# parthjaggi/flow

Hardware: AMD Instinct MI355X
Metric: env-steps/sec (higher is better)
Workload: dtype mixed

## Files before the change

flow_amd/csrc/flowsim.hip:

```cpp
#include "flowsim_sim.h"
#include "flowsim_learn.h"
#include "flowsim_es.h"

#include <cmath>

namespace fsim {

int validate(const fs_config* c) {
  if (!c) return fail(FS_ERR_INVALID, "fs_create: cfg is NULL");
  if (c->struct_size != sizeof(fs_config))
    return fail(FS_ERR_INVALID, "fs_create: struct_size mismatch (header/library out of sync)");
  if (c->abi_version != FS_ABI_VERSION) return fail(FS_ERR_INVALID, "fs_create: abi_version mismatch");
  if (c->precision != FS_F32 && c->precision != FS_F64 && c->precision != FS_MIXED && c->precision != FS_F16S)
    return fail(FS_ERR_INVALID, "fs_create: bad precision");
  if (c->precision == FS_F16S && (c->network != FS_NET_MERGE || c->num_vehicles > 64))
    return fail(FS_ERR_UNSUPPORTED, "fs_create: FS_F16S (half state, float32 integrator) is built for FS_NET_MERGE "
                                    "(k_steps_open, <= 64 vehicle slots)");
  if (c->precision == FS_MIXED && (c->network == FS_NET_MERGE || c->network == FS_NET_BOTTLENECK)) {
  } else if (c->precision == FS_MIXED) {
    const bool fig8 = c->network == FS_NET_FIGURE_EIGHT;
    const char* why = nullptr;
    if ((c->network != FS_NET_RING && !fig8) || c->num_lanes > 1) why = "network (single-lane ring or figure eight)";
    else if (c->env == FS_ENV_MULTI_WAVE_ATTENUATION_PO)
      why = "env (FS_ENV_MULTI_WAVE_ATTENUATION_PO is built for FS_F32, and for FS_F64 on the generic kernel)";
// ... 211 lines not shown
      const double x = c->init_pos[size_t(r) * c->num_vehicles + i];
      if (!(x >= 0) || !(x < L)) return fail(FS_ERR_INVALID, "fs_create: init_pos outside [0, length)");
    }
  }
  return FS_OK;
}

template <typename T>
int create_typed(const fs_config* cfg, fs_handle* out) {
  Sim<T>* s = new (std::nothrow) Sim<T>();
  if (!s) return fail(FS_ERR_HIP, "fs_create: out of host memory");
  s->cfg = *cfg;
  s->mixed = cfg->precision == FS_MIXED;
  s->f16s = cfg->precision == FS_F16S;
  s->veh.assign(cfg->vehicles, cfg->vehicles + cfg->num_vehicles);
  if (cfg->num_segments > 0) s->segs.assign(cfg->segments, cfg->segments + cfg->num_segments);
  if (cfg->obs_perm) s->obs_perm.assign(cfg->obs_perm, cfg->obs_perm + cfg->num_vehicles);
  if (cfg->network == FS_NET_MERGE || cfg->network == FS_NET_BOTTLENECK) {
    if (cfg->num_inflows > 0) s->inflows.assign(cfg->inflows, cfg->inflows + cfg->num_inflows);
    s->init_alive.assign(cfg->init_alive, cfg->init_alive + size_t(cfg->num_replicas) * cfg->num_vehicles);
    if (cfg->env == FS_ENV_BOTTLENECK_DV) {
      s->obs_cells.assign(cfg->obs_cells, cfg->obs_cells + cfg->num_obs_cells);
      if (cfg->num_rl > 0) s->act_cells.assign(cfg->act_cells, cfg->act_cells + cfg->num_rl);
    }
  }
  s->obs_dim = (cfg->env == FS_ENV_WAVE_ATTENUATION_PO) ? 3
               : (cfg->env == FS_ENV_WAVE_ATTENUATION_PO_MA) ? 3 * cfg->num_rl
               : (cfg->env == FS_ENV_MULTI_WAVE_ATTENUATION_PO) ? 3
               : (cfg->env == FS_ENV_ACCEL_PO_MA) ? 6 * cfg->num_rl
               : (cfg->env == FS_ENV_BOTTLENECK_DV) ? 4 * cfg->num_obs_cells + 1
               : (cfg->env == FS_ENV_BOTTLENECK) ? 1
               : (cfg->env == FS_ENV_MERGE_PO || cfg->env == FS_ENV_MERGE_MA)
                     ? 5 * cfg->num_rl
                     : (cfg->env == FS_ENV_LANE_CHANGE_ACCEL_PO)
                           ? (4 * (cfg->num_lanes < 1 ? 1 : cfg->num_lanes) + 1) * cfg->num_rl
                           : (cfg->env == FS_ENV_LANE_CHANGE_ACCEL ? 3 : 2) * cfg->num_vehicles;
  if (s->obs_dim < 1) s->obs_dim = 1;
  s->act_dim = cfg->num_rl * ((cfg->env == FS_ENV_LANE_CHANGE_ACCEL || cfg->env == FS_ENV_LANE_CHANGE_ACCEL_PO) ? 2 : 1);
  int seg = 8;
  while (seg < cfg->num_vehicles) seg <<= 1;
  s->seg = seg;
  hipError_t e = hipSetDevice(cfg->device);
  if (e == hipSuccess) e = hipStreamCreateWithFlags(&s->own_stream, hipStreamNonBlocking);
  if (e != hipSuccess) {
    delete s;
    return fail(FS_ERR_HIP, std::string("fs_create: no usable HIP device: ") + hipGetErrorString(e));
  }
  s->stream = s->own_stream;
  {
    const std::pair<const char*, bool SimBase::*> switches[] = {
        {"FLOWSIM_FORCE_GENERIC", &SimBase::force_generic}, {"FLOWSIM_NO_FASTDIV", &SimBase::no_fastdiv},
        {"FLOWSIM_NO_LOOP_KERNEL", &SimBase::no_loop_kernel}, {"FLOWSIM_NO_LOOP_FULL", &SimBase::no_loop_full},
        {"FLOWSIM_NO_RING_RL", &SimBase::no_ring_rl}, {"FLOWSIM_NO_QUEUE", &SimBase::no_queue},
        {"FLOWSIM_NO_PAIR", &SimBase::no_pair}, {"FLOWSIM_NO_MASK_SKIP", &SimBase::no_mask_skip},
        {"FLOWSIM_SNAPSHOT_COPIES", &SimBase::snap_copies}};
    for (const auto& sw : switches) {
      const char* v = std::getenv(sw.first);
      s->*sw.second = v && v[0] == '1';
    }
  }
  int rc = s->init();
  if (rc == FS_OK) {
    hipError_t e2 = hipStreamSynchronize(s->stream);
    if (e2 != hipSuccess) rc = fail(FS_ERR_HIP, std::string("fs_create: ") + hipGetErrorString(e2));
  }
  if (rc != FS_OK) {
    for (void* p : s->allocs) (void)hipFree(p);
    (void)hipStreamDestroy(s->own_stream);
    delete s;
    return rc;
  }
  s->cfg.vehicles = nullptr;
  s->cfg.ring_length = nullptr;
  s->cfg.init_pos = nullptr;
  s->cfg.init_vel = nullptr;
  s->cfg.init_lane = nullptr;
  s->cfg.segments = nullptr;
  s->cfg.inflows = nullptr;
  s->cfg.init_alive = nullptr;
  s->cfg.obs_cells = nullptr;
  s->cfg.obs_perm = nullptr;
  s->cfg.act_cells = nullptr;
  *out = reinterpret_cast<fs_handle>(static_cast<SimBase*>(s));
  return FS_OK;
}

inline SimBase* S(fs_handle h) { return reinterpret_cast<SimBase*>(h); }

struct DeviceGuard {
  int prev = -1;
  bool switched = false;
  explicit DeviceGuard(int want) {
    if (hipGetDevice(&prev) == hipSuccess && prev != want) switched = hipSetDevice(want) == hipSuccess;
  }
  ~DeviceGuard() {
    if (switched) (void)hipSetDevice(prev);
  }
};

}

using namespace fsim;

extern "C" {

int fs_abi_version(void) { return FS_ABI_VERSION; }

// ... 740 lines not shown
```

flow_amd/csrc/flowsim_launch.h:

```cpp
#pragma once
#include "flowsim_sim.h"
#ifdef FS_PART_QUEUE
#include "flowsim_queue.h"
#include "flowsim_dropq.h"
#endif

namespace fsim {

#ifdef FS_PART_QUEUE
  template <typename T>
  int Sim<T>::launch_queue(const StepArgs& a) {
    const bool po = dv.env == FS_ENV_MERGE_PO;
    const bool noise = (dv.flags & fs::FLAG_HAS_NOISE) != 0, act = a.actions != nullptr && (po || ov.ma_apply_actions != 0);
    const auto k = pick(noise, [&](auto NZ) {
      return pick(act, [&](auto ACT) {
        return pick(po, [&](auto PO) { return &fs::k_merge_queue<NZ, ACT, false, PO>; });
      });
    });
    last_kernel = "k_merge_queue";
    hipLaunchKernelGGL(k, dim3(dv.R), dim3(64), 0, stream, dv, ov, qc, a.num_steps, a.actions, a.act_stride, a.obs, a.rew,
                       a.done, a.obs_every_step, fs::PolicyView{}, static_cast<float*>(nullptr), static_cast<float*>(nullptr),
                       0);
    return launched();
  }
// ... 141 lines not shown
    } else if constexpr (std::is_same<T, float>::value) {
      const auto MC = std::false_type();
      k = !ma_head ? single(MC) : dv.env == FS_ENV_ACCEL_PO_MA ? kernel(Int<3>(), MC) : kernel(Int<2>(), MC);
    } else {
      k = single(std::false_type());
    }
    if constexpr (std::is_same<T, float>::value) {
      if (dv.env == FS_ENV_MULTI_WAVE_ATTENUATION_PO) k = kernel(Int<4>(), std::false_type());
    }
    last_kernel = dv.env == FS_ENV_MULTI_WAVE_ATTENUATION_PO ? "k_ring_pair<MultiRing>" : ma_head ? (dv.env == FS_ENV_ACCEL_PO_MA ? "k_ring_pair<AccelMA>" : "k_ring_pair<POMA>")
                          : (po ? "k_ring_pair<PO>" : "k_ring_pair<Accel>");
    const int waves = (dv.R + (64 / ROW) - 1) / (64 / ROW);
    hipLaunchKernelGGL(k, dim3((waves + 3) / 4), dim3(256), 0, stream, dv, a.num_steps, a.mask, a.actions, a.act_stride,
                       a.obs, a.rew, a.done, a.obs_every_step);
    return launched();
  }

  template <typename T>
  int Sim<T>::launch_obs_mixed(const StepArgs& a) {
    if constexpr (std::is_same<T, double>::value) {
      const int n = dv.R * dv.N;
      last_kernel = "k_obs_mixed";
      hipLaunchKernelGGL((fs::k_obs_mixed<T>), dim3((n + 255) / 256), dim3(256), 0, stream, dv, a.obs);
      return launched();
    } else {
      return fail(FS_ERR_UNSUPPORTED, "k_obs_mixed is a float64 kernel");
    }
  }

  template <typename T>
  template <int SEG>
  int Sim<T>::launch_pair(const StepArgs& a) {
    constexpr int ROW = SEG >= 16 ? SEG / 2 : 8;
    const bool fd = fastdiv_ok(), bc = neg_speed_possible, sm = speed_mode_any;
    const bool noise = std::is_same<T, float>::value && (dv.flags & fs::FLAG_HAS_NOISE);
    auto clamped = [&](auto SM, auto NZ) {
      return delta4 && fd && !bc ? &fs::k_rollout_pair<T, ROW, true, true, false, SM, NZ>
                                 : &fs::k_rollout_pair<T, ROW, false, false, true, SM, NZ>;
    };
    decltype(&fs::k_rollout_pair<T, ROW, false, false, true>) k = nullptr;
    if (noise) {
      if constexpr (std::is_same<T, float>::value) k = pick(sm, [&](auto SM) { return clamped(SM, std::true_type()); });
    } else if (sm) {
      k = clamped(std::true_type(), std::false_type());
    } else {
      k = pick(bc, [&](auto BC) {
        return delta4 && fd ? &fs::k_rollout_pair<T, ROW, true, true, BC>
                            : delta4 ? &fs::k_rollout_pair<T, ROW, true, false, BC> : &fs::k_rollout_pair<T, ROW, false, false, BC>;
      });
    }
    last_kernel = noise ? (sm ? "k_rollout_pair+speed_mode+noise" : "k_rollout_pair+noise")
                        : (sm ? "k_rollout_pair+speed_mode" : "k_rollout_pair");
    const int waves = (dv.R + (64 / ROW) - 1) / (64 / ROW);
    hipLaunchKernelGGL(k, dim3((waves + 3) / 4), dim3(256), 0, stream, dv, a.num_steps, a.obs, a.rew, a.done);
    return launched();
  }

  template <typename T>
  template <int SEG>
  int Sim<T>::launch_idm(const StepArgs& a) {
    constexpr int RPW = 64 / SEG;
    const bool fd = fastdiv_ok();
    const auto k = pick(neg_speed_possible, [&](auto BC) {
      return delta4 && fd ? &fs::k_rollout_idm<T, SEG, true, true, BC>
                          : delta4 ? &fs::k_rollout_idm<T, SEG, true, false, BC> : &fs::k_rollout_idm<T, SEG, false, false, BC>;
    });
    last_kernel = "k_rollout_idm";
    const int waves = (dv.R + RPW - 1) / RPW;
    hipLaunchKernelGGL(k, dim3((waves + 7) / 8), dim3(512), 0, stream, dv, a.num_steps, a.obs, a.rew, a.done, d_dump);
    return launched();
  }

  template <typename T>
  template <int SEG>
  int Sim<T>::launch_k_steps(const StepArgs& a) {
    constexpr int RPW = 64 / SEG;
    auto k = &fs::k_steps<T, SEG, 0, 0>;
    last_kernel = "k_steps";
    if (fast_ok(a)) {
      k = &fs::k_steps<T, SEG, 1, 0>;
      last_kernel = "k_steps<FAST>";
    } else if ((dv.flags & fs::FLAG_IDM_SET) && !force_generic) {
      k = &fs::k_steps<T, SEG, 0, 1>;
      last_kernel = "k_steps<CSET>";
    }
    hipLaunchKernelGGL(k, dim3((dv.R + RPW - 1) / RPW), dim3(64), 0, stream, dv, a.num_steps, a.mask, a.actions,
                       a.act_stride, a.obs, a.rew, a.done, a.obs_every_step);
    return launched();
  }

  template <typename T>
  int Sim<T>::launch_policy_act(const fs::PolicyView& pv, int n_ag, const float* obs_in, float* act, float* logp) {
    last_kernel = "k_policy_act";
    const bool merge = dv.env == FS_ENV_MERGE_MA;
    hipLaunchKernelGGL(fs::k_policy_act<16>, dim3((dv.R * 16 + 255) / 256), dim3(256), 0, stream, pv, dv.R, n_ag, dv.rep0,
                       obs_in, act, logp, merge ? static_cast<const int*>(dv.lane) : nullptr,
                       merge ? static_cast<const int*>(dv.ctrl) : nullptr,
                       merge ? static_cast<const int*>(dv.rl_index) : nullptr, dv.N);
    return launched();
  }

  template <typename T>
  int Sim<T>::launch_policy_row16(const fs::PolicyView& pv, int num_steps, int reset_done, float* obs, float* act,
                                  float* logp, float* rew, uint8_t* done) {
    const bool fast = ringrl_fast_ok();
    auto kernel = [&](auto H) {
// ... 89 lines not shown
```

flow_amd/csrc/flowsim_pair.h:

```cpp
#pragma once
#include "flowsim_kernels.h"

namespace fs {

typedef float f2 __attribute__((ext_vector_type(2)));
typedef unsigned u2v __attribute__((__vector_size__(8)));

enum : int { DPP_ROW_NEWBCAST0 = 0x150, DPP_ROW_NEWBCAST8 = 0x158 };

__device__ __forceinline__ f2 fma2(f2 a, f2 b, f2 c) { return __builtin_elementwise_fma(a, b, c); }
__device__ __forceinline__ f2 splat(float a) { return f2{a, a}; }

__device__ __forceinline__ f2 pk_mul(f2 a, f2 b) { return a * b; }
__device__ __forceinline__ f2 pk_add(f2 a, f2 b) { return a + b; }
__device__ __forceinline__ f2 pk_sub(f2 a, f2 b) { return a - b; }
__device__ __forceinline__ f2 pk_fma(f2 a, f2 b, f2 c) { return fma2(a, b, c); }
__device__ __forceinline__ f2 pk_fnma(f2 a, f2 b, f2 c) { return fma2(-a, b, c); }
__device__ __forceinline__ float nonneg_else(float x, float y) {
  const unsigned a = __builtin_bit_cast(unsigned, x), b = __builtin_bit_cast(unsigned, y);
  return __builtin_bit_cast(float, min(a, b));
}

template <int ROW>
__device__ __forceinline__ float next_a(float v, bool last, int lane) {
// ... 385 lines not shown
                                                    const MixedConsts& c) {
  unsigned long long sa, sb;
  asm volatile(
      "v_add_f64 v[134:135], v[114:115], -%[L]\n"
      "v_add_f64 v[136:137], v[116:117], -%[L]\n"
      "v_cmp_gt_i32_e64 %[sa], 0, v135\n"
      "v_cmp_gt_i32_e64 %[sb], 0, v137\n"
      "s_nop 0\n"
      "v_cndmask_b32_e64 v114, v134, v114, %[sa]\n"
      "v_cndmask_b32_e64 v115, v135, v115, %[sa]\n"
      "v_cndmask_b32_e64 v116, v136, v116, %[sb]\n"
      "v_cndmask_b32_e64 v117, v137, v117, %[sb]\n"
      "v_mul_f64 v[120:121], v[114:115], %[rcL]\n"
      "v_mul_f64 v[122:123], v[116:117], %[rcL]\n"
      "v_add_f64 v[134:135], v[116:117], -v[114:115]\n"
      "v_cvt_f32_f64_e32 v144, v[120:121]\n"
      "v_cvt_f32_f64_e32 v145, v[122:123]\n"
      "v_add_f64 v[126:127], v[134:135], %[L]\n"
      "v_mov_b32_dpp v130, v114 row_shl:1 row_mask:0xf bank_mask:0xf bound_ctrl:1\n"
      "v_mov_b32_dpp v131, v115 row_shl:1 row_mask:0xf bank_mask:0xf bound_ctrl:1\n"
      "v_mov_b32_dpp v132, v114 row_newbcast:0 row_mask:0xf bank_mask:0xf\n"
      "v_mov_b32_dpp v133, v115 row_newbcast:0 row_mask:0xf bank_mask:0xf\n"
      "v_cmp_gt_i32_e64 %[sa], 0, v135\n"
      "v_cndmask_b32_e64 v130, v130, v132, %[last]\n"
      "v_cndmask_b32_e64 v131, v131, v133, %[last]\n"
      "v_add_f64 v[136:137], v[130:131], -v[116:117]\n"
      "v_cndmask_b32_e64 v134, v134, v126, %[sa]\n"
      "v_cndmask_b32_e64 v135, v135, v127, %[sa]\n"
      "v_cndmask_b32_e64 v156, 0, %[Llo], %[sa]\n"
      "v_cndmask_b32_e64 v157, 0, %[Lhi], %[sa]\n"
      "v_add_f64 v[132:133], v[136:137], %[L]\n"
      "v_cmp_gt_i32_e64 %[sb], 0, v137\n"
      "v_add_f64 v[134:135], v[134:135], -%[lenb]\n"
      "v_cvt_f32_f64_e32 v140, v[134:135]\n"
      "v_cndmask_b32_e64 v136, v136, v132, %[sb]\n"
      "v_cndmask_b32_e64 v137, v137, v133, %[sb]\n"
      "v_cndmask_b32_e64 v158, 0, %[Llo], %[sb]\n"
      "v_cndmask_b32_e64 v159, 0, %[Lhi], %[sb]\n"
      "v_add_f64 v[136:137], v[136:137], -%[lennext]\n"
      "v_cvt_f32_f64_e32 v141, v[136:137]\n"
      "v_pk_add_f32 v[126:127], v[140:141], %[gap2] neg_lo:[0,1] neg_hi:[0,1]\n"
      "v_cmp_nlt_f32_e64 %[sa], |v140|, %[c1e3]\n"
      "v_cmp_nlt_f32_e64 %[sb], |v141|, %[c1e3]\n"
      "v_min_f32_e32 %[ct], v126, v127\n"
      "v_cndmask_b32_e64 v140, %[c1e3], v140, %[sa]\n"
      "v_cndmask_b32_e64 v141, %[c1e3], v141, %[sb]\n"
      : "+{v[114:115]}"(XA), "+{v[116:117]}"(XB), "+{v[140:141]}"(H), "+{v[144:145]}"(OX), "+{v[156:157]}"(WA),
        "+{v[158:159]}"(WB), [ct] "+v"(ct), [sa] "=&s"(sa), [sb] "=&s"(sb)
      : [L] "v"(c.L), [Llo] "v"(c.L_lo), [Lhi] "v"(c.L_hi), [rcL] "v"(c.rc_L), [gap2] "v"(c.gap2), [lenb] "v"(c.len_b),
        [lennext] "v"(c.len_next), [c1e3] "v"(c.c1e3), [last] "s"(c.last_mask)
      : "v120", "v121", "v122", "v123", "v126", "v127", "v130", "v131", "v132", "v133", "v134", "v135", "v136", "v137");
}

template <typename T, int ROW, bool DELTA4, bool FASTDIV, bool BADCHK, bool SM = false, bool NOISE = false>
__global__ __launch_bounds__(256) void k_rollout_pair(DevView<T> s, int num_steps, float* __restrict__ obs,
                                                      float* __restrict__ rew, uint8_t* __restrict__ done) {
  constexpr bool MIXED = sizeof(T) == 8;
  static_assert(!(NOISE && MIXED), "FS_MIXED has no noise form (its C twin cannot reproduce the hardware's log / cos)");
  constexpr bool ASM = ROW == 16 && DELTA4 && FASTDIV && !BADCHK;
  constexpr int RPW = 64 / ROW;
  constexpr int PERIOD = ROW < 16 ? ROW : 16;
  const int lane = threadIdx.x & 63;
  const int wave = (blockIdx.x * blockDim.x + threadIdx.x) >> 6;
  const int row = lane / ROW;
  const int k = lane % ROW;
  const int r = wave * RPW + row;
  const int N = s.N;
  const int LP = N >> 1;
  const bool rvalid = r < s.R;
  const bool valid = rvalid && k < LP;
  const int rr = rvalid ? r : s.R - 1;
  const int kk = k < LP ? k : LP - 1;
  const bool last = (kk == LP - 1);
  const int iA = 2 * kk, iB = iA + 1;
  const size_t idx = size_t(rr) * N + iA;

  f2 p[6];
#pragma unroll
  for (int q = 0; q < 6; ++q) p[q] = f2{float(s.p[q * N + iA]), float(s.p[q * N + iB])};
  const T lenB = s.length[iB];
  const T len_nextA = next_a<ROW>(T(s.length[iA]), last, lane);
  const T base_len = s.ring_len[rr];
  const T L = base_len + T(4) * s.jlen;
  int tcount = s.time[rr];
  uint32_t nctr = NOISE ? s.noise_ctr[rr] : 0u;
  const f2 sigma = NOISE ? f2{float(s.noise[iA]), float(s.noise[iB])} : f2{0.0f, 0.0f};
  const bool noisyA = NOISE && sigma.x > 0.0f, noisyB = NOISE && sigma.y > 0.0f;
  float gA[4] = {0.0f, 0.0f, 0.0f, 0.0f}, gB[4] = {0.0f, 0.0f, 0.0f, 0.0f};
  if constexpr (NOISE) {
    if ((nctr & 3u) != 0u) {
      gauss4<float>(s.seed_lo, s.seed_hi, s.rep0 + uint32_t(rr), uint32_t(iA), nctr >> 2, gA, s.noise_exact != 0);
      gauss4<float>(s.seed_lo, s.seed_hi, s.rep0 + uint32_t(rr), uint32_t(iB), nctr >> 2, gB, s.noise_exact != 0);
      for (uint32_t q = 0; q < (nctr & 3u); ++q) {
        gA[0] = gA[1]; gA[1] = gA[2]; gA[2] = gA[3];
        gB[0] = gB[1]; gB[1] = gB[2]; gB[2] = gB[3];
      }
    }
  }

  const float dt = float(s.dt), ramp = float(s.ramp);
  const f2 two_sqrt_ab = {2.0f * tsqrt(p[2].x * p[3].x), 2.0f * tsqrt(p[2].y * p[3].y)};
  const f2 rc_v0 = {1.0f / p[0].x, 1.0f / p[0].y}, rc_ab = {1.0f / two_sqrt_ab.x, 1.0f / two_sqrt_ab.y};
  const float Lf = float(L);
  const f2 L2 = splat(Lf), rc_L2 = splat(1.0f / Lf), one = splat(1.0f), dt2 = splat(dt), ramp2 = splat(ramp);
  const f2 gap2 = splat(float(s.crash_gap)), m100 = splat(-100.0f);
  const f2 vmask = splat(valid ? 1.0f : 0.0f), tvm = splat(valid ? -float(s.target_velocity) : 0.0f);
  const double ms64 = double(s.max_speed), rc_ms64 = 1.0 / ms64;
  const double L64 = double(L), rc_L64 = 1.0 / L64, dt64 = double(s.dt), ramp64 = double(s.ramp);

  f2 x, v;
  double xdA = 0, xdB = 0, vdA = 0, vdB = 0;
  if (MIXED) {
    xdA = double(s.pos[idx]); xdB = double(s.pos[idx + 1]);
    vdA = double(s.vel[idx]); vdB = double(s.vel[idx + 1]);
    v = f2{float(vdA), float(vdB)};
    x = f2{0.0f, 0.0f};
  } else {
    x = f2{float(s.pos[idx]), float(s.pos[idx + 1])};
    v = f2{float(s.vel[idx]), float(s.vel[idx + 1])};
  }
// ... 27 lines not shown
  mc.p0 = p[0]; mc.p1 = p[1]; mc.p2 = p[2]; mc.p5 = p[5]; mc.rc_v0 = rc_v0; mc.tsab = two_sqrt_ab; mc.rc_ab = rc_ab;
  mc.one = one; mc.gap2 = gap2; mc.vmask = vmask; mc.tvm = tvm; mc.c1e3 = 1e-3f; mc.dt = dt64; mc.ramp = ramp64;
  mc.L = L64; mc.rc_L = rc_L64; mc.rc_ms = rc_ms64; mc.len_b = double(lenB); mc.len_next = double(len_nextA);
  mc.zero = 0.0; mc.last_mask = pc.last_mask;
  {
    const unsigned long long Lb = __builtin_bit_cast(unsigned long long, L64);
    mc.L_lo = unsigned(Lb); mc.L_hi = unsigned(Lb >> 32);
    mc.thr = mc.L_hi < 0x457CED91u ? mc.L_hi : 0x457CED91u;
  }
  double wA = 0.0, wB = 0.0;
  if constexpr (ASM && MIXED) {
    asm volatile("" : "+v"(mc.dt), "+v"(mc.ramp), "+v"(mc.one), "+v"(mc.zero), "+v"(mc.rc_ms), "+v"(mc.c1e3), "+v"(mc.gap2));
    const double xn = next_a<ROW>(xdA, last, lane);
    wA = xdB - xdA < 0.0 ? L64 : 0.0;
    wB = xn - xdB < 0.0 ? L64 : 0.0;
    h.x = tabs(h.x) < 1e-3f ? 1e-3f : h.x;
    h.y = tabs(h.y) < 1e-3f ? 1e-3f : h.y;
  }
  SumoPair sc{};
  double floor0A = 0, floor0B = 0, adtA = 0, adtB = 0, ddtA = 0, ddtB = 0;
  if constexpr (SM) {
    const int mA = s.speed_mode[iA], mB = s.speed_mode[iB];
    const float maA = float(s.max_accel[iA]), maB = float(s.max_accel[iB]);
    const float mdA = float(s.max_decel[iA]), mdB = float(s.max_decel[iB]);
    sc.tau = f2{float(s.sumo_tau[iA]), float(s.sumo_tau[iB])};
    sc.min_gap = f2{float(s.sumo_min_gap[iA]), float(s.sumo_min_gap[iB])};
    sc.maxa = f2{maA, maB};
    sc.smax = f2{float(s.sumo_max_speed[iA]), float(s.sumo_max_speed[iB])};
    sc.rc_smax = f2{1.0f / sc.smax.x, 1.0f / sc.smax.y};
    sc.ts = f2{2.0f * tsqrt(maA * mdA), 2.0f * tsqrt(maB * mdB)};
    sc.rc_ts = f2{1.0f / sc.ts.x, 1.0f / sc.ts.y};
    const float BIG = 3.0e38f;
    sc.floor0 = f2{(mA & 1) ? 0.0f : BIG, (mB & 1) ? 0.0f : BIG};
    sc.adt = f2{(mA & 2) ? maA * dt : BIG, (mB & 2) ? maB * dt : BIG};
    sc.ddt = f2{(mA & 4) ? mdA * dt : BIG, (mB & 4) ? mdB * dt : BIG};
    floor0A = double(sc.floor0.x); floor0B = double(sc.floor0.y);
    adtA = (mA & 2) ? double(s.max_accel[iA]) * dt64 : double(BIG);
    adtB = (mB & 2) ? double(s.max_accel[iB]) * dt64 : double(BIG);
    ddtA = (mA & 4) ? double(s.max_decel[iA]) * dt64 : double(BIG);
    ddtB = (mB & 4) ? double(s.max_decel[iB]) * dt64 : double(BIG);
  }
  const MixedSumoConsts msc = {floor0A, floor0B, adtA, adtB, ddtA, ddtB};

  const unsigned rowb = 2u * unsigned(N) * 4u;
  const unsigned off_v = unsigned(rr) * rowb + unsigned(iA) * 4u;
  const unsigned off_x = off_v + unsigned(N) * 4u;
  const size_t step_bytes = size_t(s.R) * rowb;
  const unsigned step_b32 = unsigned(step_bytes);
  char* ob = reinterpret_cast<char*>(obs);
  unsigned crash_bits = 0u, bad_bits = 0u;

  typedef unsigned u4v __attribute__((__vector_size__(16)));
  constexpr bool XPOSE = ASM;
  __shared__ float row_img[XPOSE ? 4 : 1][XPOSE ? RPW * 64 : 1];
  float* const my_img = row_img[XPOSE ? (threadIdx.x >> 6) & 3 : 0] + (XPOSE ? row * 2 * N : 0);
  const unsigned off_16 = unsigned(rr) * rowb + unsigned(kk) * 16u;
  u4v piece = {0u, 0u, 0u, 0u};
  auto transpose_in = [&](f2 ov, f2 ox) {
    *reinterpret_cast<f2*>(my_img + 2 * kk) = ov;
    *reinterpret_cast<f2*>(my_img + N + 2 * kk) = ox;
    __builtin_amdgcn_fence(__ATOMIC_RELEASE, "wavefront");
    __builtin_amdgcn_wave_barrier();
    __builtin_amdgcn_fence(__ATOMIC_ACQUIRE, "wavefront");
    piece = *reinterpret_cast<const u4v*>(my_img + 4 * kk);
  };

  auto noise_term = [&]() -> f2 {
    f2 nz = {-0.0f, -0.0f};
    if constexpr (NOISE) {
      const bool fresh = (nctr & 3u) == 0u;
      if (__ballot(fresh) != 0ull) {
        if (fresh) {
          gauss4<float>(s.seed_lo, s.seed_hi, s.rep0 + uint32_t(rr), uint32_t(iA), nctr >> 2, gA, s.noise_exact != 0);
          gauss4<float>(s.seed_lo, s.seed_hi, s.rep0 + uint32_t(rr), uint32_t(iB), nctr >> 2, gB, s.noise_exact != 0);
        }
      }
      const float tA = sigma.x * gA[0], tB = sigma.y * gB[0];
      nz.x = noisyA ? tA : -0.0f;
      nz.y = noisyB ? tB : -0.0f;
      gA[0] = gA[1]; gA[1] = gA[2]; gA[2] = gA[3];
      gB[0] = gB[1]; gB[1] = gB[2]; gB[2] = gB[3];
      nctr += 1u;
    }
    return nz;
  };

  auto one_step = [&](int slot, __amdgpu_buffer_rsrc_t rs, float& sq_out) {
    if constexpr (ASM) {
      f2 ov, ox;
      const unsigned so = unsigned(slot) * step_b32;
      if constexpr (MIXED) {
        if constexpr (SM) mixed_step_asm_a_sm(v, xdA, xdB, vdA, vdB, h, dvl, ov, mc, sc, msc);
        else mixed_step_asm_a(v, xdA, xdB, vdA, vdB, h, dvl, ov, mc);
        if (slot > 0) __builtin_amdgcn_raw_buffer_store_b128(piece, rs, off_16, so - step_b32, 0);
        float ct;
        unsigned long long need;
        mixed_step_asm_b(v, xdA, xdB, h, dvl, ox, wA, wB, ct, sq_out, need, mc);
#if defined(FS_DIAG_ALWAYS_SLOW)
        need = ~0ull;
#elif defined(FS_DIAG_NEVER_SLOW)
        need = 0ull;
#endif
        if (__builtin_expect(need != 0ull, 0)) mixed_step_asm_slow(xdA, xdB, h, ox, wA, wB, ct, mc);
        crash_bits = __builtin_amdgcn_alignbit(crash_bits, __builtin_bit_cast(unsigned, ct), 31);
        transpose_in(ov, ox);
      } else {
#if defined(FS_DIAG_NOSTORE)
        pair_step_asm_a(v, x, h, dvl, ox, pc);
        pair_step_asm_b(v, x, h, dvl, ov, crash_bits, sq_out, pc);
        asm volatile("" :: "v"(ov), "v"(ox), "s"(so));
#elif defined(FS_DIAG_NOXPOSE)
        pair_step_asm_a(v, x, h, dvl, ox, pc);
        __builtin_amdgcn_raw_buffer_store_b64(__builtin_bit_cast(u2v, ox), rs, off_x, so, 0);
        pair_step_asm_b(v, x, h, dvl, ov, crash_bits, sq_out, pc);
        __builtin_amdgcn_raw_buffer_store_b64(__builtin_bit_cast(u2v, ov), rs, off_v, so, 0);
#else
        if constexpr (NOISE) {
          const f2 nz = noise_term();
          if constexpr (SM) pair_step_asm_a_sm_nz(v, x, h, dvl, ox, pc, sc, nz);
          else pair_step_asm_a_nz(v, x, h, dvl, ox, pc, nz);
        } else {
          if constexpr (SM) pair_step_asm_a_sm(v, x, h, dvl, ox, pc, sc);
          else pair_step_asm_a(v, x, h, dvl, ox, pc);
        }
        if (slot > 0) __builtin_amdgcn_raw_buffer_store_b128(piece, rs, off_16, so - step_b32, 0);
        pair_step_asm_b(v, x, h, dvl, ov, crash_bits, sq_out, pc);
        transpose_in(ov, ox);
#endif
      }
      return;
    }
    f2 acc = idm_pair<DELTA4, FASTDIV>(v, vl, h, p, two_sqrt_ab, rc_ab, rc_v0, one);
    if constexpr (NOISE) acc = pk_add(acc, noise_term());
    f2 acc_s = {0.0f, 0.0f};
    if constexpr (SM) acc_s = sumo_acc_pair<FASTDIV>(v, vl, h, sc, one);
    f2 ox;
    if (MIXED) {
      const double aA = double(acc.x), aB = double(acc.y);
      const double nA = tmax(vdA + aA * dt64, 0.0), nB = tmax(vdB + aB * dt64, 0.0);
      double cA = vdA + (nA - vdA) * ramp64, cB = vdB + (nB - vdB) * ramp64;
      if constexpr (SM) {
        const double sA = tmax(vdA + double(acc_s.x) * dt64, floor0A), sB = tmax(vdB + double(acc_s.y) * dt64, floor0B);
        cA = tmin(cA, sA); cB = tmin(cB, sB);
        cA = tmin(cA, vdA + adtA); cB = tmin(cB, vdB + adtB);
        cA = tmax(cA, vdA - ddtA); cB = tmax(cB, vdB - ddtB);
      }
      vdA = cA;
      vdB = cB;
      const double xA = xdA + vdA * dt64, xB = xdB + vdB * dt64;
      xdA = xA >= L64 ? xA - L64 : xA;
      xdB = xB >= L64 ? xB - L64 : xB;
      v = f2{float(vdA), float(vdB)};
      ox = f2{float(xdA * rc_L64), float(xdB * rc_L64)};
    } else {
      f2 nv = pk_add(v, pk_mul(acc, dt2));
      nv.x = tmax(nv.x, 0.0f);
      nv.y = tmax(nv.y, 0.0f);
      f2 vc = pk_add(v, pk_mul(pk_sub(nv, v), ramp2));
      if constexpr (SM) {
        const f2 vs = pk_add(v, pk_mul(acc_s, dt2));
        const f2 cap1 = pk_add(v, sc.adt), flo = pk_sub(v, sc.ddt);
        vc.x = tmin(vc.x, tmax(sc.floor0.x, vs.x));
        vc.y = tmin(vc.y, tmax(sc.floor0.y, vs.y));
        vc.x = tmax(tmin(vc.x, cap1.x), flo.x);
        vc.y = tmax(tmin(vc.y, cap1.y), flo.y);
      }
      v = vc;
      const f2 xn = pk_add(x, pk_mul(v, dt2));
      const f2 xw = pk_sub(xn, L2);
      x.x = nonneg_else(xw.x, xn.x);
      x.y = nonneg_else(xw.y, xn.y);
      ox = div_const2<FASTDIV>(x, L2, rc_L2);
    }
    h = headway();
    vl = f2{v.y, next_a<ROW>(v.x, last, lane)};
    const f2 hc = pk_sub(h, gap2);
    crash_bits = __builtin_amdgcn_alignbit(crash_bits, __builtin_bit_cast(unsigned, __builtin_fminf(hc.x, hc.y)), 31);
    if (BADCHK) {
      const f2 vb = pk_sub(v, m100);
      bad_bits = __builtin_amdgcn_alignbit(bad_bits, __builtin_bit_cast(unsigned, __builtin_fminf(vb.x, vb.y)), 31);
    }
    f2 ov;
    if (MIXED) ov = f2{float(vdA * rc_ms64), float(vdB * rc_ms64)};
    else ov = f2{div_via_f64(v.x, ms64, rc_ms64), div_via_f64(v.y, ms64, rc_ms64)};
    const unsigned so = unsigned(slot) * step_b32;
    __builtin_amdgcn_raw_buffer_store_b64(__builtin_bit_cast(u2v, ov), rs, off_v, so, 0);
    __builtin_amdgcn_raw_buffer_store_b64(__builtin_bit_cast(u2v, ox), rs, off_x, so, 0);
    const f2 dv = pk_fma(v, vmask, tvm);
    const f2 sq = pk_mul(dv, dv);
    sq_out = sq.x + sq.y;
  };

  int base = 0;
  for (; base + PERIOD <= num_steps; base += PERIOD) {
    float sq[PERIOD];
    const size_t remain = size_t(num_steps - base) * step_bytes;
    const __amdgpu_buffer_rsrc_t rs = __builtin_amdgcn_make_buffer_rsrc(
        ob, 0, remain > 0xFFFFFFFFull ? 0xFFFFFFFFu : unsigned(remain), 0x00020000);
#pragma unroll
    for (int slot = 0; slot < PERIOD; ++slot) one_step(slot, rs, sq[slot]);
#if !defined(FS_DIAG_NOSTORE) && !defined(FS_DIAG_NOXPOSE)
    if (XPOSE) __builtin_amdgcn_raw_buffer_store_b128(piece, rs, off_16, unsigned(PERIOD - 1) * step_b32, 0);
#endif
    ob += size_t(PERIOD) * step_bytes;
    tcount += PERIOD;
    const float racc = transposed_sum<ROW, PERIOD>(sq, lane);
    const unsigned crash_any = seg_or<ROW>(crash_bits);
    const unsigned bad_any = (BADCHK ? seg_or<ROW>(bad_bits) : 0u) | crash_any;
    crash_bits = 0u;
    bad_bits = 0u;
    if (rvalid && k < PERIOD) {
      const bool my_crash = (crash_any >> (PERIOD - 1 - k)) & 1u;
      const bool my_bad = (bad_any >> (PERIOD - 1 - k)) & 1u;
      const int t_k = tcount - (PERIOD - 1 - k);
      const float cost = tsqrt(racc);
      const float max_cost = float(s.max_cost);
      float reward = tmax(max_cost - cost, 0.0f) / (max_cost + 1.1920928955078125e-07f);
      reward = my_bad ? 0.0f : reward;
      const size_t o = size_t(base + k) * s.R + rr;
      rew[o] = reward;
      done[o] = done_flag(t_k >= s.step_limit, my_crash);
    }
  }
#pragma unroll 1
  for (; base < num_steps; ++base) {
    float sq1;
    const __amdgpu_buffer_rsrc_t rs = __builtin_amdgcn_make_buffer_rsrc(ob, 0, unsigned(step_bytes), 0x00020000);
    one_step(0, rs, sq1);
#if !defined(FS_DIAG_NOSTORE) && !defined(FS_DIAG_NOXPOSE)
    if (XPOSE) __builtin_amdgcn_raw_buffer_store_b128(piece, rs, off_16, 0u, 0);
#endif
    ob += step_bytes;
    tcount += 1;
    const float racc = seg_sum<ROW>(sq1);
    const bool my_crash = (seg_or<ROW>(crash_bits) & 1u) != 0u;
    const bool my_bad = (BADCHK && (seg_or<ROW>(bad_bits) & 1u) != 0u) || my_crash;
    crash_bits = 0u;
    bad_bits = 0u;
    if (rvalid && k == 0) {
      const float cost = tsqrt(racc);
      const float max_cost = float(s.max_cost);
      float reward = tmax(max_cost - cost, 0.0f) / (max_cost + 1.1920928955078125e-07f);
      reward = my_bad ? 0.0f : reward;
      const size_t o = size_t(base) * s.R + rr;
      rew[o] = reward;
      done[o] = done_flag(tcount >= s.step_limit, my_crash);
    }
  }
  if (valid) {
    if (MIXED) {
      s.pos[idx] = T(xdA); s.pos[idx + 1] = T(xdB);
      s.vel[idx] = T(vdA); s.vel[idx + 1] = T(vdB);
    } else {
      s.pos[idx] = T(x.x); s.pos[idx + 1] = T(x.y);
      s.vel[idx] = T(v.x); s.vel[idx + 1] = T(v.y);
    }
    if (kk == 0) s.time[rr] = tcount;
    if (NOISE && kk == 0) s.noise_ctr[rr] = nctr;
  }
}

template <typename T>
__global__ void k_obs_mixed(DevView<T> s, float* __restrict__ obs) {
  if constexpr (std::is_same<T, double>::value) {
    const int e = blockIdx.x * blockDim.x + threadIdx.x;
    if (e >= s.R * s.N) return;
    const int r = e / s.N, i = e % s.N;
    const double L = s.ring_len[r] + 4.0 * s.jlen;
    float* o = obs + size_t(r) * 2 * s.N;
    o[i] = float(s.vel[e] * (1.0 / double(s.max_speed)));
    o[s.N + i] = float(s.pos[e] * (1.0 / L));
  }
}

}
```

flow_amd/csrc/flowsim_sim.h:

```cpp
#pragma once
#include <hip/hip_runtime.h>

#include <algorithm>
#include <climits>
#include <cmath>
#include <cstdio>
#include <cstdlib>
#include <cstring>
#include <map>
#include <mutex>
#include <new>
#include <string>
#include <type_traits>
#include <vector>

#include "flowsim.h"
#include "flowsim_kernels.h"
#include "flowsim_open.h"
#include "flowsim_pair.h"
#include "flowsim_fig8.h"
#include "flowsim_ringrl.h"
#include "flowsim_policy.h"
#include "flowsim_wide.h"
#include "flowsim_queue_consts.h"
// ... 12 lines not shown
#define HIP_TRY(expr)                                                                      \
  do {                                                                                     \
    hipError_t e_ = (expr);                                                                \
    if (e_ != hipSuccess)                                                                  \
      return fail(FS_ERR_HIP, std::string(#expr) + " failed: " + hipGetErrorString(e_));   \
  } while (0)

struct StepArgs {
  int num_steps;
  const uint8_t* mask;
  const float* actions;
  size_t act_stride;
  float* obs;
  float* rew;
  uint8_t* done;
  int obs_every_step;
};

template <int N>
using Int = std::integral_constant<int, N>;

template <typename F>
auto pick(bool b, F&& f) {
  return b ? f(std::true_type()) : f(std::false_type());
}

struct SimBase {
  virtual ~SimBase() {}
  fs_config cfg{};
  std::vector<fs_vehicle_spec> veh;
  std::vector<fs_segment> segs;
  std::vector<fs_inflow> inflows;
  std::vector<fs_cell> obs_cells, act_cells;
  std::vector<int32_t> obs_perm;
  std::vector<uint8_t> init_alive;
  int obs_dim = 0;
  int act_dim = 0;
  int seg = 0;
  hipStream_t own_stream = nullptr;
  hipStream_t stream = nullptr;
  float* d_actions = nullptr;
  float* d_obs = nullptr;
  float* d_rew = nullptr;
  uint8_t* d_done = nullptr;
  uint8_t* d_mask = nullptr;
  float* d_dump = nullptr;
  std::vector<void*> allocs;
  int after_reset = 0;
  bool force_generic = false;
  bool no_fastdiv = false;
  bool f16s = false;
  bool mixed = false;
  bool no_pair = false;
  bool no_loop_kernel = false;
  bool no_loop_full = false;
  bool no_ring_rl = false;
  bool no_mask_skip = false;
  bool no_queue = false;
  bool snap_copies = false;
  double* d_ep_scratch = nullptr;
  double* d_adv_scratch = nullptr;
  unsigned* d_mb_ticket = nullptr;
  int* d_qflag = nullptr;
  bool qflag_armed = false;
  int check_qflag() {
    if (!qflag_armed || !d_qflag) return FS_OK;
    int f = 0;
    HIP_TRY(hipMemcpy(&f, d_qflag, sizeof(int), hipMemcpyDeviceToHost));
    if (f != 0)
      return fail(FS_ERR_UNSUPPORTED, "k_drop_queue: a path of the lane-drop network held more than 64 vehicles (or more than 8 "
                                      "arrived in one sub-step): the results of this handle are invalid -- create it "
                                      "with FLOWSIM_NO_QUEUE=1 (slot-order kernels)");
    qflag_armed = false;
    return FS_OK;
  }
  bool has_user_ctrl = false;
  const char* last_kernel = "";
  int launched() {
    HIP_TRY(hipGetLastError());
    return FS_OK;
  }

  virtual int launch_steps(int num_steps, const uint8_t* mask, const float* actions, size_t act_stride,
                           float* obs, float* rew, uint8_t* done, int obs_every_step) = 0;
  virtual int launch_reset(const uint8_t* mask) = 0;
  virtual int launch_policy(const fs_policy* pol, int num_steps, int reset_done, const float* obs_in, float* obs,
                            float* act, float* logp, float* rew, uint8_t* done) = 0;
  virtual int launch_policy_pair(const fs_policy* av, const fs_policy* adv, float pw, int num_steps, int reset_done,
                                 const float* obs_in, float* obs, float* act, float* logp, float* cmd, float* rew,
                                 uint8_t* done) = 0;
  virtual int launch_population(const fs_policy* pol, const fs_population* pop, int probe, int num_steps, int reset_done,
                                const float* obs_in, float* obs, float* act, float* logp, float* rew, uint8_t* done) = 0;
  std::string last_kernel_pop;
  unsigned* d_es_ticket = nullptr;
  uint32_t* d_pol_ctr = nullptr;
  fs::SnapTable snap{};
  size_t snap_bytes = 0;
  uint64_t snap_layout = 0;
  uint64_t snap_nonce = 0;
  virtual void snap_mirrors_out() = 0;
  virtual void snap_mirrors_in() = 0;
  virtual void snap_mirrors_blob(const char* dev_part) = 0;
  virtual int get_state(int field, void* dst, size_t bytes) = 0;
  virtual int set_state(int field, const void* src, size_t bytes) = 0;
  virtual int add_vehicle(int replica, int slot, int route, double x, double speed) = 0;
};
// ... 1329 lines not shown
```

Baseline: 13.93 billion.

## Add N=22 specialized pair kernel with LDS ring buffer for observation stores

Adds a k_rollout_pair_n variant specialized at compile time for 22 vehicles (11 lane pairs). It stages a full 16-step observation image in LDS as a ring and writes it back as whole-wave 16-byte pieces during the next period, replacing the per-step partial-row transpose stores. The goal is better coalesced global writes and fewer per-step store/transpose overheads, and a compile-time N also lets the compiler specialize the arithmetic. In exchange it uses more LDS per wave and adds deferred-store bookkeeping. It is dispatched only for runs of 512 or more steps unless an env switch overrides that.

```diff
diff --git a/flow_amd/csrc/flowsim.hip b/flow_amd/csrc/flowsim.hip
--- a/flow_amd/csrc/flowsim.hip
+++ b/flow_amd/csrc/flowsim.hip
@@ -287,7 +287,9 @@
         {"FLOWSIM_FORCE_GENERIC", &SimBase::force_generic}, {"FLOWSIM_NO_FASTDIV", &SimBase::no_fastdiv},
         {"FLOWSIM_NO_LOOP_KERNEL", &SimBase::no_loop_kernel}, {"FLOWSIM_NO_LOOP_FULL", &SimBase::no_loop_full},
         {"FLOWSIM_NO_RING_RL", &SimBase::no_ring_rl}, {"FLOWSIM_NO_QUEUE", &SimBase::no_queue},
-        {"FLOWSIM_NO_PAIR", &SimBase::no_pair}, {"FLOWSIM_NO_MASK_SKIP", &SimBase::no_mask_skip},
+        {"FLOWSIM_NO_PAIR", &SimBase::no_pair}, {"FLOWSIM_PAIR_GENERIC_N", &SimBase::pair_generic_n},
+        {"FLOWSIM_KERNEL_DETAIL", &SimBase::kernel_detail}, {"FLOWSIM_PAIR_N_ALWAYS", &SimBase::pair_n_always},
+        {"FLOWSIM_NO_MASK_SKIP", &SimBase::no_mask_skip},
         {"FLOWSIM_SNAPSHOT_COPIES", &SimBase::snap_copies}};
     for (const auto& sw : switches) {
       const char* v = std::getenv(sw.first);
diff --git a/flow_amd/csrc/flowsim_launch.h b/flow_amd/csrc/flowsim_launch.h
--- a/flow_amd/csrc/flowsim_launch.h
+++ b/flow_amd/csrc/flowsim_launch.h
@@ -217,6 +217,21 @@
     last_kernel = noise ? (sm ? "k_rollout_pair+speed_mode+noise" : "k_rollout_pair+noise")
                         : (sm ? "k_rollout_pair+speed_mode" : "k_rollout_pair");
     const int waves = (dv.R + (64 / ROW) - 1) / (64 / ROW);
+    if constexpr (SEG == 32) {
+      if (dv.N == 22 && delta4 && fd && !bc && !pair_generic_n && (a.num_steps >= PAIR_N_MIN_STEPS || pair_n_always)) {
+        decltype(&fs::k_rollout_pair_n<T, 11>) kn = nullptr;
+        if constexpr (std::is_same<T, float>::value) {
+          kn = pick(sm, [&](auto SM) { return pick(noise, [&](auto NZ) { return &fs::k_rollout_pair_n<T, 11, SM, NZ>; }); });
+        } else {
+          kn = pick(sm, [&](auto SM) { return &fs::k_rollout_pair_n<T, 11, SM>; });
+        }
+        if (kernel_detail)
+          last_kernel = noise ? (sm ? "k_rollout_pair+speed_mode+noise[n11]" : "k_rollout_pair+noise[n11]")
+                              : (sm ? "k_rollout_pair+speed_mode[n11]" : "k_rollout_pair[n11]");
+        hipLaunchKernelGGL(kn, dim3((waves + 3) / 4), dim3(256), 0, stream, dv, a.num_steps, a.obs, a.rew, a.done);
+        return launched();
+      }
+    }
     hipLaunchKernelGGL(k, dim3((waves + 3) / 4), dim3(256), 0, stream, dv, a.num_steps, a.obs, a.rew, a.done);
     return launched();
   }
diff --git a/flow_amd/csrc/flowsim_pair.h b/flow_amd/csrc/flowsim_pair.h
--- a/flow_amd/csrc/flowsim_pair.h
+++ b/flow_amd/csrc/flowsim_pair.h
@@ -461,9 +461,14 @@
       : "v120", "v121", "v122", "v123", "v126", "v127", "v130", "v131", "v132", "v133", "v134", "v135", "v136", "v137");
 }
 
-template <typename T, int ROW, bool DELTA4, bool FASTDIV, bool BADCHK, bool SM = false, bool NOISE = false>
-__global__ __launch_bounds__(256) void k_rollout_pair(DevView<T> s, int num_steps, float* __restrict__ obs,
-                                                      float* __restrict__ rew, uint8_t* __restrict__ done) {
+template <typename F, int... S>
+__device__ __forceinline__ void each_slot(F&& f, std::integer_sequence<int, S...>) {
+  (f(std::integral_constant<int, S>()), ...);
+}
+
+template <typename T, int ROW, bool DELTA4, bool FASTDIV, bool BADCHK, bool SM, bool NOISE, int NH>
+__device__ __forceinline__ void rollout_pair_body(const DevView<T>& s, int num_steps, float* __restrict__ obs,
+                                                  float* __restrict__ rew, uint8_t* __restrict__ done) {
   constexpr bool MIXED = sizeof(T) == 8;
   static_assert(!(NOISE && MIXED), "FS_MIXED has no noise form (its C twin cannot reproduce the hardware's log / cos)");
   constexpr bool ASM = ROW == 16 && DELTA4 && FASTDIV && !BADCHK;
@@ -474,7 +479,7 @@
   const int row = lane / ROW;
   const int k = lane % ROW;
   const int r = wave * RPW + row;
-  const int N = s.N;
+  const int N = NH > 0 ? 2 * NH : s.N;
   const int LP = N >> 1;
   const bool rvalid = r < s.R;
   const bool valid = rvalid && k < LP;
@@ -608,8 +613,32 @@
 
   typedef unsigned u4v __attribute__((__vector_size__(16)));
   constexpr bool XPOSE = ASM;
-  __shared__ float row_img[XPOSE ? 4 : 1][XPOSE ? RPW * 64 : 1];
-  float* const my_img = row_img[XPOSE ? (threadIdx.x >> 6) & 3 : 0] + (XPOSE ? row * 2 * N : 0);
+  constexpr bool RING = ASM && NH > 0
+#if defined(FS_DIAG_PAIRN_NO_RING)
+      && false
+#endif
+      ;
+#if defined(FS_DIAG_PAIRN_BURST)
+  constexpr bool BURST = true;
+#else
+  constexpr bool BURST = false;
+#endif
+  constexpr int WSTEP = RPW * 8 * (NH > 0 ? 2 * NH : 1);
+  constexpr int NPIECE = NH > 0 ? NH : 1;
+  static_assert(!RING || (PERIOD * WSTEP == NPIECE * 1024 && WSTEP <= 1024), "the 16-step image is NPIECE full-wave pieces");
+  __shared__ __attribute__((aligned(16))) float row_img[XPOSE ? 4 : 1][RING ? PERIOD * WSTEP / 4 : XPOSE ? RPW * 64 : 1];
+  float* const my_wave_img = row_img[XPOSE ? (threadIdx.x >> 6) & 3 : 0];
+  float* const my_img = my_wave_img + (XPOSE ? row * 2 * N : 0);
+  unsigned doff[NPIECE];
+  if constexpr (RING) {
+#pragma unroll
+    for (int j = 0; j < NPIECE; ++j) {
+      const unsigned g = unsigned(j) * 1024u + 16u * unsigned(lane);
+      const unsigned st = g / unsigned(WSTEP), in_step = g % unsigned(WSTEP);
+      const int rp = wave * RPW + int(in_step / rowb);
+      doff[j] = st * step_b32 + unsigned(rp < s.R ? rp : s.R - 1) * rowb + in_step % rowb;
+    }
+  }
   const unsigned off_16 = unsigned(rr) * rowb + unsigned(kk) * 16u;
   u4v piece = {0u, 0u, 0u, 0u};
   auto transpose_in = [&](f2 ov, f2 ox) {
@@ -619,6 +648,39 @@
     __builtin_amdgcn_wave_barrier();
     __builtin_amdgcn_fence(__ATOMIC_ACQUIRE, "wavefront");
     piece = *reinterpret_cast<const u4v*>(my_img + 4 * kk);
+  };
+  typedef __attribute__((address_space(3))) char lds_char;
+  typedef __attribute__((address_space(3))) f2 lds_f2;
+  constexpr int WR_SPAN = RING ? (255 * 8 - 4 * 2 * NH) / WSTEP + 1 : PERIOD;
+  constexpr int WR_BASES = (PERIOD + WR_SPAN - 1) / WR_SPAN;
+  lds_char* ring_wr[WR_BASES] = {};
+  if constexpr (RING) {
+#pragma unroll
+    for (int q = 0; q < WR_BASES; ++q) {
+      ring_wr[q] = (lds_char*)(reinterpret_cast<char*>(my_img + 2 * kk)) + q * WR_SPAN * WSTEP;
+      asm volatile("" : "+v"(ring_wr[q]));
+    }
+  }
+  const char* const ring_rd = reinterpret_cast<const char*>(my_wave_img + 4 * lane);
+#if defined(FS_DIAG_PAIRN_NO_MERGE)
+  const int wr_dist = 4 * s.N;
+#else
+  constexpr int wr_dist = 4 * (NH > 0 ? 2 * NH : 1);
+#endif
+  auto ring_piece = [&](int j) { return *reinterpret_cast<const u4v*>(ring_rd + j * 1024); };
+  auto ring_in = [&](int slot, f2 ov, f2 ox) {
+    if (!BURST && slot < NPIECE) {
+      piece = ring_piece(slot);
+      __builtin_amdgcn_fence(__ATOMIC_RELEASE, "wavefront");
+      __builtin_amdgcn_wave_barrier();
+      __builtin_amdgcn_fence(__ATOMIC_ACQUIRE, "wavefront");
+    }
+    lds_char* const at = ring_wr[slot / WR_SPAN] + (slot % WR_SPAN) * WSTEP;
+    *(lds_f2*)at = ov;
+    *(lds_f2*)(at + wr_dist) = ox;
+    __builtin_amdgcn_fence(__ATOMIC_RELEASE, "wavefront");
+    __builtin_amdgcn_wave_barrier();
+    __builtin_amdgcn_fence(__ATOMIC_ACQUIRE, "wavefront");
   };
 
   auto noise_term = [&]() -> f2 {
@@ -641,14 +703,26 @@
     return nz;
   };
 
-  auto one_step = [&](int slot, __amdgpu_buffer_rsrc_t rs, float& sq_out) {
+  auto one_step = [&](int slot, __amdgpu_buffer_rsrc_t rs, float& sq_out, auto IN_RING, __amdgpu_buffer_rsrc_t rs_prev)
+                      __attribute__((always_inline)) {
     if constexpr (ASM) {
       f2 ov, ox;
       const unsigned so = unsigned(slot) * step_b32;
+      auto store_late = [&]() {
+        if constexpr (decltype(IN_RING)::value) {
+          if (!BURST && slot >= 1 && slot <= NPIECE) __builtin_amdgcn_raw_buffer_store_b128(piece, rs_prev, doff[slot - 1], 0, 0);
+        } else {
+          if (slot > 0) __builtin_amdgcn_raw_buffer_store_b128(piece, rs, off_16, so - step_b32, 0);
+        }
+      };
+      auto rows_in = [&]() {
+        if constexpr (decltype(IN_RING)::value) ring_in(slot, ov, ox);
+        else transpose_in(ov, ox);
+      };
       if constexpr (MIXED) {
         if constexpr (SM) mixed_step_asm_a_sm(v, xdA, xdB, vdA, vdB, h, dvl, ov, mc, sc, msc);
         else mixed_step_asm_a(v, xdA, xdB, vdA, vdB, h, dvl, ov, mc);
-        if (slot > 0) __builtin_amdgcn_raw_buffer_store_b128(piece, rs, off_16, so - step_b32, 0);
+        store_late();
         float ct;
         unsigned long long need;
         mixed_step_asm_b(v, xdA, xdB, h, dvl, ox, wA, wB, ct, sq_out, need, mc);
@@ -659,7 +733,7 @@
 #endif
         if (__builtin_expect(need != 0ull, 0)) mixed_step_asm_slow(xdA, xdB, h, ox, wA, wB, ct, mc);
         crash_bits = __builtin_amdgcn_alignbit(crash_bits, __builtin_bit_cast(unsigned, ct), 31);
-        transpose_in(ov, ox);
+        rows_in();
       } else {
 #if defined(FS_DIAG_NOSTORE)
         pair_step_asm_a(v, x, h, dvl, ox, pc);
@@ -679,9 +753,9 @@
           if constexpr (SM) pair_step_asm_a_sm(v, x, h, dvl, ox, pc, sc);
           else pair_step_asm_a(v, x, h, dvl, ox, pc);
         }
-        if (slot > 0) __builtin_amdgcn_raw_buffer_store_b128(piece, rs, off_16, so - step_b32, 0);
+        store_late();
         pair_step_asm_b(v, x, h, dvl, ov, crash_bits, sq_out, pc);
-        transpose_in(ov, ox);
+        rows_in();
 #endif
       }
       return;
@@ -748,15 +822,37 @@
   };
 
   int base = 0;
+  char* ob_prev = ob;
+  unsigned prev_bytes = 0u;
+  const std::integral_constant<bool, RING> in_ring{};
   for (; base + PERIOD <= num_steps; base += PERIOD) {
     float sq[PERIOD];
     const size_t remain = size_t(num_steps - base) * step_bytes;
     const __amdgpu_buffer_rsrc_t rs = __builtin_amdgcn_make_buffer_rsrc(
         ob, 0, remain > 0xFFFFFFFFull ? 0xFFFFFFFFu : unsigned(remain), 0x00020000);
+    const __amdgpu_buffer_rsrc_t rs_prev = __builtin_amdgcn_make_buffer_rsrc(ob_prev, 0, prev_bytes, 0x00020000);
+    if constexpr (RING) {
+      each_slot([&](auto S) __attribute__((always_inline)) { one_step(S.value, rs, sq[S.value], in_ring, rs_prev); },
+                std::make_integer_sequence<int, PERIOD>());
+    } else {
 #pragma unroll
-    for (int slot = 0; slot < PERIOD; ++slot) one_step(slot, rs, sq[slot]);
+      for (int slot = 0; slot < PERIOD; ++slot) one_step(slot, rs, sq[slot], in_ring, rs_prev);
+    }
 #if !defined(FS_DIAG_NOSTORE) && !defined(FS_DIAG_NOXPOSE)
-    if (XPOSE) __builtin_amdgcn_raw_buffer_store_b128(piece, rs, off_16, unsigned(PERIOD - 1) * step_b32, 0);
+    if constexpr (RING) {
+      if constexpr (BURST) {
+#pragma unroll
+        for (int j = 0; j < NPIECE; ++j) __builtin_amdgcn_raw_buffer_store_b128(ring_piece(j), rs, doff[j], 0, 0);
+        __builtin_amdgcn_fence(__ATOMIC_RELEASE, "wavefront");
+        __builtin_amdgcn_wave_barrier();
+        __builtin_amdgcn_fence(__ATOMIC_ACQUIRE, "wavefront");
+      } else {
+        ob_prev = ob;
+        prev_bytes = unsigned(PERIOD) * step_b32;
+      }
+    } else if (XPOSE) {
+      __builtin_amdgcn_raw_buffer_store_b128(piece, rs, off_16, unsigned(PERIOD - 1) * step_b32, 0);
+    }
 #endif
     ob += size_t(PERIOD) * step_bytes;
     tcount += PERIOD;
@@ -778,11 +874,19 @@
       done[o] = done_flag(t_k >= s.step_limit, my_crash);
     }
   }
+  if (RING && !BURST && prev_bytes != 0u) {
+    const __amdgpu_buffer_rsrc_t rs_prev = __builtin_amdgcn_make_buffer_rsrc(ob_prev, 0, prev_bytes, 0x00020000);
+#pragma unroll
+    for (int j = 0; j < NPIECE; ++j) __builtin_amdgcn_raw_buffer_store_b128(ring_piece(j), rs_prev, doff[j], 0, 0);
+    __builtin_amdgcn_fence(__ATOMIC_RELEASE, "wavefront");
+    __builtin_amdgcn_wave_barrier();
+    __builtin_amdgcn_fence(__ATOMIC_ACQUIRE, "wavefront");
+  }
 #pragma unroll 1
   for (; base < num_steps; ++base) {
     float sq1;
     const __amdgpu_buffer_rsrc_t rs = __builtin_amdgcn_make_buffer_rsrc(ob, 0, unsigned(step_bytes), 0x00020000);
-    one_step(0, rs, sq1);
+    one_step(0, rs, sq1, std::false_type(), rs);
 #if !defined(FS_DIAG_NOSTORE) && !defined(FS_DIAG_NOXPOSE)
     if (XPOSE) __builtin_amdgcn_raw_buffer_store_b128(piece, rs, off_16, 0u, 0);
 #endif
@@ -816,6 +920,18 @@
   }
 }
 
+template <typename T, int ROW, bool DELTA4, bool FASTDIV, bool BADCHK, bool SM = false, bool NOISE = false>
+__global__ __launch_bounds__(256) void k_rollout_pair(DevView<T> s, int num_steps, float* __restrict__ obs,
+                                                      float* __restrict__ rew, uint8_t* __restrict__ done) {
+  rollout_pair_body<T, ROW, DELTA4, FASTDIV, BADCHK, SM, NOISE, 0>(s, num_steps, obs, rew, done);
+}
+template <typename T, int NH, bool SM = false, bool NOISE = false>
+__global__ __launch_bounds__(256) void k_rollout_pair_n(DevView<T> s, int num_steps, float* __restrict__ obs,
+                                                        float* __restrict__ rew, uint8_t* __restrict__ done) {
+  static_assert(NH >= 1 && NH <= 16, "a row of 16 lanes holds up to 32 vehicles");
+  rollout_pair_body<T, 16, true, true, false, SM, NOISE, NH>(s, num_steps, obs, rew, done);
+}
+
 template <typename T>
 __global__ void k_obs_mixed(DevView<T> s, float* __restrict__ obs) {
   if constexpr (std::is_same<T, double>::value) {
diff --git a/flow_amd/csrc/flowsim_sim.h b/flow_amd/csrc/flowsim_sim.h
--- a/flow_amd/csrc/flowsim_sim.h
+++ b/flow_amd/csrc/flowsim_sim.h
@@ -88,6 +88,10 @@
   bool f16s = false;
   bool mixed = false;
   bool no_pair = false;
+  bool pair_generic_n = false;
+  bool pair_n_always = false;
+  static constexpr int PAIR_N_MIN_STEPS = 512;
+  bool kernel_detail = false;
   bool no_loop_kernel = false;
   bool no_loop_full = false;
   bool no_ring_rl = false;
```

Result: faster. 14.99 billion, median of 6 (+7.6%).
